# Keep-Passion/ImageStitch

Measured on AMD Instinct MI355X. Metric: image-pairs/sec (2048x2048 grayscale, SURF+BF), higher is better.
Workload: dtype f32

## Files before the change

### imagestitch_amd/csrc/surf_kernels.hip

```cpp
#include "common.h"
#include "detmath.h"
#include <math.h>
#include <float.h>
#include <string.h>
#include <stdlib.h>
#include <algorithm>
#include <vector>

#define GAS __attribute__((address_space(1)))
typedef GAS const uint8_t *g_cu8;
typedef GAS const int32_t *g_ci32;
typedef GAS float *g_f32;
typedef GAS const float *g_cf32;
typedef GAS int32_t *g_i32;
__device__ __forceinline__ int cv_round_f(float v) { return (int)rintf(v); }
__device__ __forceinline__ uint8_t round_u8_pos(float v) { return (uint8_t)__float_as_uint(v + 12582912.f); }
__device__ __forceinline__ int cv_round_d(double v) { return (int)rint(v); }
__device__ __forceinline__ int cv_floor_d(double v) { return (int)floor(v); }
__device__ __forceinline__ int cv_ceil_d(double v) { return (int)ceil(v); }

__device__ __forceinline__ int wave_incl_scan(int v)
{
    const int lane = threadIdx.x & 63;
#pragma unroll
// ... 730 lines not shown
        if (a1 > me.k1) rank++;
        else if (a1 == me.k1) {
            const unsigned long long a2 = S[q].k2, a3 = S[q].k3;
            rank += (a2 < me.k2 || (a2 == me.k2 && a3 < me.k3)) ? 1 : 0;
        }
    }
    const Cand c = R.cand[me.idx];
    vfsms_keypoint kp;
    kp.x = c.x; kp.y = c.y; kp.size = c.size; kp.angle = -1.f; kp.response = c.response;
    kp.octave = c.octave; kp.class_id = cand_class_id(R, pats, c);
    R.kps[rank] = kp;
}

__device__ __forceinline__ float fast_atan2_deg(float y, float x)
{
    const float s = (float)(180 / 3.1415926535897932384626433832795);
    const float p1 = 0.9997878412794807f * s, p3 = -0.3258083974640975f * s;
    const float p5 = 0.1555786518463281f * s, p7 = -0.04432655554792128f * s;
    float ax = fabsf(x), ay = fabsf(y);
    float a, c, c2;
    if (ax >= ay) {
        c = ay / (ax + (float)DBL_EPSILON);
        c2 = c * c;
        a = (((p7 * c2 + p5) * c2 + p3) * c2 + p1) * c;
    } else {
        c = ax / (ay + (float)DBL_EPSILON);
        c2 = c * c;
        a = 90.f - (((p7 * c2 + p5) * c2 + p3) * c2 + p1) * c;
    }
    if (x < 0) a = 180.f - a;
    if (y < 0) a = 360.f - a;
    return a;
}

#ifndef ORI_KP
#define ORI_KP 2
#endif
typedef float ori_f2 __attribute__((ext_vector_type(2)));
__device__ __forceinline__ void orientation_block(const RoiDev &R, const SurfTables *T, const int k0, const int n, int upright)
{
    __shared__ __attribute__((aligned(16))) float2 XY[ORI_KP][128];
    __shared__ __attribute__((aligned(16))) uint8_t Zb[ORI_KP][9][128];
    __shared__ float mod_s[ORI_KP][72], sx_s[ORI_KP][72], sy_s[ORI_KP][72];
    __shared__ int nvalid[ORI_KP], state[ORI_KP];
    const int tid = threadIdx.x;
    const int kq = __builtin_amdgcn_readfirstlane(tid >> 7), t = tid & 127;
    if (tid < ORI_KP) { nvalid[tid] = 0; state[tid] = 0; }
    __syncthreads();
    {
        const int k = k0 + kq;
        int valid = 0;
        uint32_t m0 = 0, m1 = 0, m2 = 0;
        float2 xy = make_float2(0.f, 0.f);
        if (k < n) {
            const vfsms_keypoint kp = R.kps[k];
            const float s = kp.size * 1.2f / 9.0f;
            const int gws = 2 * cv_round_f(2 * s);
            const int srows = R.h + 1, scols = R.w + 1, sw = R.w + 1;
            if (srows < gws || scols < gws) {
                if (t == 0) { R.kps[k].size = -1.f; state[kq] = 1; }
            } else if (upright) {
                if (t == 0) { R.kps[k].angle = 270.f; state[kq] = 1; }
            } else if (t < T->nOriSamples) {
                int x = cv_round_f(kp.x + T->aptx[t] * s - (float)(gws - 1) / 2);
                int y = cv_round_f(kp.y + T->apty[t] * s - (float)(gws - 1) / 2);
                if (!(y < 0 || y >= srows - gws || x < 0 || x >= scols - gws)) {
                    const float ratio = (float)gws / 4;
                    const int r2 = cv_round_f(ratio * 2), r4 = cv_round_f(ratio * 4);
                    g_ci32 p0 = (g_ci32)R.sum + (size_t)y * sw + x;
                    g_ci32 p2 = p0 + (size_t)r2 * sw, p4 = p0 + (size_t)r4 * sw;
                    const int a00 = p0[0], a02 = p0[r2], a04 = p0[r4];
                    const int a20 = p2[0], a24 = p2[r4];
                    const int a40 = p4[0], a42 = p4[r2], a44 = p4[r4];
                    const float wA = 1.f / ((float)r2 * (float)r4);
                    float wB = wA;
                    if (r4 - r2 != r2) wB = 1.f / ((float)(r4 - r2) * (float)r4);
                    const int vx0 = a00 + a42 - a40 - a02, vx1 = a02 + a44 - a42 - a04;
                    const int vy0 = a00 + a24 - a20 - a04, vy1 = a20 + a44 - a40 - a24;
                    double dxd = 0; dxd += (double)(-((float)vx0 * wA)); dxd += (double)((float)vx1 * wB);
                    double dyd = 0; dyd += (double)((float)vy0 * wA); dyd += (double)(-((float)vy1 * wB));
                    const float vx = (float)dxd, vy = (float)dyd;
                    const float aw = T->aptw[t];
                    const float xx = vx * aw, yy = vy * aw;
                    xy = make_float2(xx, yy);
                    const int ang = cv_round_f(fast_atan2_deg(yy, xx));
                    const uint32_t *mrow = T->oriMask[min(max(ang, 0), 360)];
                    m0 = mrow[0]; m1 = mrow[1]; m2 = mrow[2];
                    valid = 1;
                }
            }
        } else if (t == 0) state[kq] = 1;
        XY[kq][t] = xy;
        Zb[kq][0][t] = (uint8_t)m0; Zb[kq][1][t] = (uint8_t)(m0 >> 8); Zb[kq][2][t] = (uint8_t)(m0 >> 16); Zb[kq][3][t] = (uint8_t)(m0 >> 24);
        Zb[kq][4][t] = (uint8_t)m1; Zb[kq][5][t] = (uint8_t)(m1 >> 8); Zb[kq][6][t] = (uint8_t)(m1 >> 16); Zb[kq][7][t] = (uint8_t)(m1 >> 24);
        Zb[kq][8][t] = (uint8_t)m2;
        const unsigned long long m = __ballot(valid);
        if ((tid & 63) == 0 && m) atomicAdd(&nvalid[kq], __popcll(m));
    }
    __syncthreads();
    if (tid < ORI_KP * 72) {
        const int q = tid / 72, w = tid - q * 72;
        if (state[q] == 0 && nvalid[q] > 0) {
            const int nori = T->nOriSamples;
            const uint8_t *zrow = Zb[q][w >> 3];
            const int bit = w & 7;
            ori_f2 acc = {0.f, 0.f};
            for (int j = 0; j < nori; j += 8) {
                const uint2 z8 = *reinterpret_cast<const uint2 *>(&zrow[j]);
                const uint32_t za = (z8.x >> bit) & 0x01010101u, zb = (z8.y >> bit) & 0x01010101u;
                const float4 p01 = *reinterpret_cast<const float4 *>(&XY[q][j]), p23 = *reinterpret_cast<const float4 *>(&XY[q][j + 2]);
                const float4 p45 = *reinterpret_cast<const float4 *>(&XY[q][j + 4]), p67 = *reinterpret_cast<const float4 *>(&XY[q][j + 6]);
#define ORI_ACC(Z, N, P, XC, YC) do { float mf; asm("v_cvt_f32_ubyte" #N " %0, %1" : "=v"(mf) : "v"(Z)); \
                                           acc = __builtin_elementwise_fma((ori_f2){P.XC, P.YC}, (ori_f2){mf, mf}, acc); } while (0)
                ORI_ACC(za, 0, p01, x, y); ORI_ACC(za, 1, p01, z, w); ORI_ACC(za, 2, p23, x, y); ORI_ACC(za, 3, p23, z, w);
                ORI_ACC(zb, 0, p45, x, y); ORI_ACC(zb, 1, p45, z, w); ORI_ACC(zb, 2, p67, x, y); ORI_ACC(zb, 3, p67, z, w);
#undef ORI_ACC
            }
            const float sumx = acc.x, sumy = acc.y;
            mod_s[q][w] = sumx * sumx + sumy * sumy;
            sx_s[q][w] = sumx; sy_s[q][w] = sumy;
        }
    }
    __syncthreads();
    {
        const int q = __builtin_amdgcn_readfirstlane(tid >> 6), lane = tid & 63;
        if (q < ORI_KP && state[q] == 0) {
            const int k = k0 + q;
            if (nvalid[q] == 0) {
                if (lane == 0) R.kps[k].size = -1.f;
            } else {
                float bm = mod_s[q][lane]; int bi = lane;
                if (!(bm > 0.f)) bm = 0.f;
                if (lane < 8) { float m2 = mod_s[q][64 + lane]; if (m2 > bm) { bm = m2; bi = 64 + lane; } }
#pragma unroll
                for (int off = 32; off >= 1; off >>= 1) {
                    const float om = __shfl_xor(bm, off, 64); const int oi = __shfl_xor(bi, off, 64);
                    if (om > bm || (om == bm && oi < bi)) { bm = om; bi = oi; }
                }
                if (lane == 0) {
                    float bestx = 0, besty = 0;
                    if (bm > 0.f) { bestx = sx_s[q][bi]; besty = sy_s[q][bi]; }
                    R.kps[k].angle = fast_atan2_deg(-besty, bestx);
                }
            }
        }
    }
}

#ifdef VFSMS_DESC_TIMING
__device__ unsigned long long g_desc_cycles[8];
#define DT_MARK(ph) do { if (threadIdx.x == 0) { unsigned long long _n = clock64(); atomicAdd(&g_desc_cycles[ph], _n - _t0); _t0 = _n; } } while (0)
#define DT_START unsigned long long _t0 = clock64()
extern "C" int vfsms_debug_desc_cycles(unsigned long long *out) { return hipMemcpyFromSymbol(out, HIP_SYMBOL(g_desc_cycles), sizeof(unsigned long long) * 8) == hipSuccess ? 0 : -3; }
__device__ unsigned long long g_desc_trips[4];
#define DT_TRIP(n) do {} while (0)
__device__ unsigned long long g_desc_unit_cycles[4];
#define DT_UNIT_BEGIN unsigned long long _u0 = clock64()
#define DT_UNIT_END(n) do { _uacc[n] += clock64() - _u0; _ucnt[n]++; } while (0)
extern "C" int vfsms_debug_desc_unit_cycles(unsigned long long *out) { return hipMemcpyFromSymbol(out, HIP_SYMBOL(g_desc_unit_cycles), sizeof(unsigned long long) * 4) == hipSuccess ? 0 : -3; }
extern "C" int vfsms_debug_desc_trips(unsigned long long *out) { return hipMemcpyFromSymbol(out, HIP_SYMBOL(g_desc_trips), sizeof(unsigned long long) * 4) == hipSuccess ? 0 : -3; }
#else
#define DT_MARK(ph) do {} while (0)
#define DT_START do {} while (0)
#define DT_TRIP(n) do {} while (0)
#define DT_UNIT_BEGIN do {} while (0)
#define DT_UNIT_END(n) do {} while (0)
#endif
#ifndef VFSMS_EXP
#define VFSMS_EXP 0
#endif
#ifndef DESC_WBUF
#define DESC_WBUF 15360
#endif
__device__ __forceinline__ void origin_chain(float *row, float s, const float d, const int n)
{
    int i = 0;
    for (; i + 4 <= n; i += 4) {
        const float a = s, b = a + d, c = b + d, e = c + d;
        s = e + d;
        row[i] = a; row[i + 1] = b; row[i + 2] = c; row[i + 3] = e;
    }
    for (; i < n; i++, s += d) row[i] = s;
}

struct WinGeom {
    int win; float sin_dir, cos_dir;
    int h, w, stride; g_cu8 img;
    g_cu8 pair;
    int upright, usx, usy;
};

__device__ __forceinline__ int win_sample_xy(const WinGeom &G, double px, double py)
{
    const int ncols1 = G.w - 1, nrows1 = G.h - 1;
    const int ix = (int)px, iy = (int)py;
    if (px >= 0.0 && py >= 0.0 && ix < ncols1 && iy < nrows1) {
        const float a = (float)__builtin_amdgcn_fract(px), b = (float)__builtin_amdgcn_fract(py);
        g_cu8 p = G.img + (size_t)iy * G.stride + ix;
        const float v = p[0] * (1.f - a) * (1.f - b) + p[1] * a * (1.f - b) + p[G.stride] * (1.f - a) * b + p[G.stride + 1] * a * b;
        return (int)(uint8_t)cv_round_f(v);
    }
    const int x = min(max(cv_round_d(px), 0), ncols1);
    const int y = min(max(cv_round_d(py), 0), nrows1);
    return (int)G.img[(size_t)y * G.stride + x];
}
__device__ __forceinline__ int win_sample_upright(const WinGeom &G, int i, int j)
{
    const int x = min(max(G.usx + i, 0), G.w - 1);
    const int y = min(max(G.usy - j, 0), G.h - 1);
    return (int)G.img[(size_t)y * G.stride + x];
}

typedef float float2v __attribute__((ext_vector_type(2)));
__device__ __forceinline__ float bilinear_pk(uint32_t top, float a, float b)
{
    const float na = 1.f - a, nb = 1.f - b;
    const float2v w = {na, a};
    const float2v r0 = {(float)(top & 0xff), (float)((top >> 16) & 0xff)};
    const float2v r1 = {(float)((top >> 8) & 0xff), (float)(top >> 24)};
    float2v p = r0 * w, q = r1 * w;
    const float2v nb2 = {nb, nb}, b2 = {b, b};
    p = p * nb2; q = q * b2;
    return ((p.x + p.y) + q.x) + q.y;
}
#ifndef STAGE_ILP
#define STAGE_ILP 4
#endif
#define UNIT_W (8 * STAGE_ILP)
#ifndef BORDER_ILP
#define BORDER_ILP 2
#endif
#ifndef STAGE_FRAC_FIRST
#define STAGE_FRAC_FIRST 1
#endif
template <int N>
__device__ __forceinline__ void stage_round(g_cu8 ubase, const uint32_t pw, const double c, const double sn, const double sxc, const double syc,
                                            const int jlane, uint8_t *wrow)
{
    uint32_t top[N];
    const double jd = (double)jlane;
    const double px0 = __builtin_fma(jd, c, sxc), py0 = __builtin_fma(jd, -sn, syc);
#if STAGE_FRAC_FIRST
    float fa[N], fb[N];
#pragma unroll
    for (int u = 0; u < N; u++) {
        const double px = u ? px0 + (double)(8 * u) * c : px0, py = u ? py0 - (double)(8 * u) * sn : py0;
        const uint32_t off = ((uint32_t)__umul24((uint32_t)(int)py, pw) + (uint32_t)(int)px) << 1;
        fa[u] = (float)__builtin_amdgcn_fract(px); fb[u] = (float)__builtin_amdgcn_fract(py);
        top[u] = *(GAS const uint32_t *)(ubase + off);
    }
#pragma unroll
    for (int u = 0; u < N; u++) wrow[8 * u] = round_u8_pos(bilinear_pk(top[u], fa[u], fb[u]));
#else
    double px[N], py[N];
    px[0] = px0; py[0] = py0;
#pragma unroll
    for (int u = 1; u < N; u++) { px[u] = px[0] + (double)(8 * u) * c; py[u] = py[0] - (double)(8 * u) * sn; }
#pragma unroll
    for (int u = 0; u < N; u++) {
        const uint32_t off = ((uint32_t)__umul24((uint32_t)(int)py[u], pw) + (uint32_t)(int)px[u]) << 1;
        top[u] = *(GAS const uint32_t *)(ubase + off);
    }
#pragma unroll
    for (int u = 0; u < N; u++) {
        const float a = (float)__builtin_amdgcn_fract(px[u]), b = (float)__builtin_amdgcn_fract(py[u]);
        wrow[8 * u] = round_u8_pos(bilinear_pk(top[u], a, b));
    }
#endif
}

template <int NW>
__device__ __forceinline__ void stage_rows(const WinGeom &G, const float *sx_row, const float *sy_row,
                                           int r0, int nrows, uint8_t *dst, uint8_t *strip_in)
{
    const int win = __builtin_amdgcn_readfirstlane(G.win);
    r0 = __builtin_amdgcn_readfirstlane(r0); nrows = __builtin_amdgcn_readfirstlane(nrows);
    const int lane = threadIdx.x & 63, wv = NW == 1 ? 0 : __builtin_amdgcn_readfirstlane((int)(threadIdx.x >> 6));
    const int li = lane >> 3, lj = lane & 7;
    const int strips = (nrows + 7) >> 3;
    const double c = (double)G.cos_dir, sn = (double)G.sin_dir;
    const int ncols1 = __builtin_amdgcn_readfirstlane(G.w) - 1, nrows1 = __builtin_amdgcn_readfirstlane(G.h) - 1;
    const uint64_t bp = (uint64_t)G.pair;
    g_cu8 ubase = (g_cu8)(((uint64_t)(uint32_t)__builtin_amdgcn_readfirstlane((uint32_t)(bp >> 32)) << 32) |
                          (uint64_t)(uint32_t)__builtin_amdgcn_readfirstlane((uint32_t)bp));
    const uint32_t pw = (uint32_t)(ncols1 + 1);
    const int gfull = win >> 3, tailc = win & 7;
    int nb = NW == 1 ? 1 : (gfull + 7) >> 3;
#if VFSMS_EXP & 16
    nb = (gfull + 3) >> 2;
#endif
    const int gbase = gfull / nb, grem = gfull - gbase * nb;
    const int total = strips * nb;
    if (!G.upright) {
        const int tid = NW == 1 ? lane : (int)threadIdx.x;
        if (tid < strips) {
            const int ia = min(r0 + tid * 8, VFSMS_MAX_WIN - 1), ib = min(min(r0 + tid * 8 + 7, r0 + nrows - 1), VFSMS_MAX_WIN - 1);
            const double xa = (double)sx_row[ia], xb = (double)sx_row[ib], ya = (double)sy_row[ia], yb = (double)sy_row[ib];
            const double jb = (double)(win - 1);
            const double jxb = jb * c, jyb = -(jb * sn);
            const double xmin = fmin(xa, xb) + fmin(0.0, jxb), xmax = fmax(xa, xb) + fmax(0.0, jxb);
            const double ymin = fmin(ya, yb) + fmin(0.0, jyb), ymax = fmax(ya, yb) + fmax(0.0, jyb);
            strip_in[tid] = xmin >= 0.0 && ymin >= 0.0 && xmax < (double)(ncols1 - 2) && ymax < (double)nrows1;
        }
        if (NW == 1) { __builtin_amdgcn_fence(__ATOMIC_ACQ_REL, "wavefront"); __builtin_amdgcn_wave_barrier(); }
        else __syncthreads();
    }
    int ty = 0, cbi = wv;
    while (cbi >= nb) { cbi -= nb; ty++; }
#ifdef VFSMS_DESC_TIMING
    unsigned long long _s0 = clock64(), _uacc[2] = {0, 0}, _ucnt[2] = {0, 0};
#endif
    const int last_row = r0 + nrows - 1;
    const int liw = li * win;
    const int last_off = (nrows - 1) * win;
    float nsx = 0.f, nsy = 0.f; int nflag = 0;
    if (wv < total) {
        const int ic0 = min(r0 + ty * 8 + li, last_row);
        nsx = sx_row[ic0]; nsy = sy_row[ic0]; nflag = strip_in[ty];
    }
    for (int unit = wv; unit < total; unit += NW) {
        DT_UNIT_BEGIN;
        const int g0 = cbi * gbase + min(cbi, grem), gn = gbase + (cbi < grem ? 1 : 0);
        const bool last_run = cbi == nb - 1;
        const int cb0 = g0 * 8;
        const int cb1 = last_run ? win : cb0 + gn * 8;
        const double sxc = (double)nsx, syc = (double)nsy;
        const int flag_cur = nflag;
        const int ty_cur = ty;
        uint8_t *drc = dst + min(ty * 8 * win + liw, last_off);
        cbi += NW;
        while (cbi >= nb) { cbi -= nb; ty++; }
        if (unit + NW < total) {
            const int icn = min(r0 + ty * 8 + li, last_row);
            nsx = sx_row[icn]; nsy = sy_row[icn]; nflag = strip_in[ty];
        }
        if (G.upright) {
            for (int j = cb0 + lj; j < cb1; j += 8) drc[j] = (uint8_t)win_sample_upright(G, min(r0 + ty_cur * 8 + li, last_row), j);
            continue;
        }
        bool unit_in = __builtin_amdgcn_readfirstlane(flag_cur) != 0;
        if (!unit_in) {
            const int ia = min(r0 + ty_cur * 8, VFSMS_MAX_WIN - 1), ib = min(min(r0 + ty_cur * 8 + 7, last_row), VFSMS_MAX_WIN - 1);
            const double xa = (double)sx_row[ia], xb = (double)sx_row[ib], ya = (double)sy_row[ia], yb = (double)sy_row[ib];
            const double ja = (double)cb0, jb = (double)(cb1 - 1);
            const double jxa = ja * c, jxb = jb * c, jya = -(ja * sn), jyb = -(jb * sn);
            const double xmin = fmin(xa, xb) + fmin(jxa, jxb), xmax = fmax(xa, xb) + fmax(jxa, jxb);
            const double ymin = fmin(ya, yb) + fmin(jya, jyb), ymax = fmax(ya, yb) + fmax(jya, jyb);
            unit_in = xmin >= 0.0 && ymin >= 0.0 && xmax < (double)(ncols1 - 2) && ymax < (double)nrows1;
        }
        if (unit_in) {
            DT_TRIP(0);
            uint8_t *wrow = drc + cb0 + lj;
            int jl = cb0 + lj, left = gn;
            while (left >= 4) { stage_round<4>(ubase, pw, c, sn, sxc, syc, jl, wrow); jl += 32; wrow += 32; left -= 4; }
            if (left == 3) stage_round<3>(ubase, pw, c, sn, sxc, syc, jl, wrow);
            else if (left == 2) stage_round<2>(ubase, pw, c, sn, sxc, syc, jl, wrow);
            else if (left == 1) stage_round<1>(ubase, pw, c, sn, sxc, syc, jl, wrow);
            if (last_run && tailc) {
                const int jc = min(gfull * 8 + lj, win - 1);
                stage_round<1>(ubase, pw, c, sn, sxc, syc, jc, drc + jc);
            }
            DT_UNIT_END(0);
            continue;
        }
        DT_TRIP(2);
        for (int jb = cb0; jb < cb1; jb += 8 * BORDER_ILP) {
            double px[BORDER_ILP], py[BORDER_ILP];
            int jc[BORDER_ILP];
            uint32_t top[BORDER_ILP];
            bool inside[BORDER_ILP];
#pragma unroll
            for (int u = 0; u < BORDER_ILP; u++) {
                jc[u] = min(jb + u * 8 + lj, cb1 - 1);
                px[u] = sxc + (double)jc[u] * c;
                py[u] = syc - (double)jc[u] * sn;
                const int ix = (int)px[u], iy = (int)py[u];
                inside[u] = px[u] >= 0.0 && py[u] >= 0.0 && ix < ncols1 && iy < nrows1;
                const int rx = min(max(cv_round_d(px[u]), 0), ncols1), ry = min(max(cv_round_d(py[u]), 0), nrows1);
                const int cx = inside[u] ? ix : rx, cy = inside[u] ? iy : ry;
                top[u] = *(GAS const uint32_t *)(ubase + (((uint32_t)__umul24((uint32_t)cy, pw) + (uint32_t)cx) << 1));
            }
#pragma unroll
            for (int u = 0; u < BORDER_ILP; u++) {
                const float a = (float)__builtin_amdgcn_fract(px[u]), b = (float)__builtin_amdgcn_fract(py[u]);
                const float v = (float)(top[u] & 0xff) * (1.f - a) * (1.f - b) + (float)((top[u] >> 16) & 0xff) * a * (1.f - b) +
                                (float)((top[u] >> 8) & 0xff) * (1.f - a) * b + (float)(top[u] >> 24) * a * b;
                drc[jc[u]] = inside[u] ? (uint8_t)cv_round_f(v) : (uint8_t)(top[u] & 0xff);
            }
        }
        DT_UNIT_END(1);
    }
#ifdef VFSMS_DESC_TIMING
    if ((threadIdx.x & 63) == 0) {
        atomicAdd(&g_desc_unit_cycles[2], clock64() - _s0);
        atomicAdd(&g_desc_unit_cycles[0], _uacc[0]); atomicAdd(&g_desc_unit_cycles[1], _uacc[1]);
        atomicAdd(&g_desc_trips[0], _ucnt[0]); atomicAdd(&g_desc_trips[2], _ucnt[1]);
    }
#endif
}

__device__ __forceinline__ uint8_t sat_u8(float v)
{
    int iv = cv_round_f(v);
    return (uint8_t)(iv < 0 ? 0 : iv > 255 ? 255 : iv);
}

struct AreaRec { int j0, n; float a0, af, al; int mode, r1, r2; };
#define AREA_RECS 22

__device__ __forceinline__ float area_row_tab(const uint8_t *S, const AreaRec &c, const int nmin, const int nmax)
{
    const uint8_t *p = S + c.j0;
    float buf = (float)p[0] * c.a0;
    int t = 1;
    for (; t < nmin - 1; t++) buf += (float)p[t] * c.af;
    for (; t < nmax; t++) buf += (float)p[t] * (t < c.n - 1 ? c.af : (t == c.n - 1 ? c.al : 0.f));
    return buf;
}
#define AREA_TAIL 4
__device__ __forceinline__ void area_tail_weights(const AreaRec &c, const int nmin, float (&w)[AREA_TAIL])
{
    const int t0 = max(nmin - 1, 1);
#pragma unroll
    for (int i = 0; i < AREA_TAIL; i++) w[i] = t0 + i < c.n - 1 ? c.af : (t0 + i == c.n - 1 ? c.al : 0.f);
}
__device__ __forceinline__ float area_row_tab_w(const uint8_t *S, const AreaRec &c, const int nmin, const int nmax, const float (&w)[AREA_TAIL])
{
    const uint8_t *p = S + c.j0;
    float buf = (float)p[0] * c.a0;
    int t = 1;
    for (; t < nmin - 1; t++) buf += (float)p[t] * c.af;
#pragma unroll
    for (int i = 0; i < AREA_TAIL; i++)
        if (t + i < nmax) buf += (float)p[t + i] * w[i];
    return buf;
}
__device__ __forceinline__ uint8_t area_out(const float sum, const int mode, const float inv_area)
{
    if (mode == 2) return (uint8_t)(((int)sum + 2) >> 2);
    if (mode == 1) return sat_u8(sum * inv_area);
    return sat_u8(sum);
}
__device__ __forceinline__ uint8_t area_col_tab(const float *rb, const AreaRec &c, const int mode, const float inv_area)
{
    float sum = c.a0 * rb[0];
    for (int t = 1; t < c.n; t++) sum += (t < c.n - 1 ? c.af : c.al) * rb[t * 21];
    return area_out(sum, mode, inv_area);
}
#define DESC_ACC_OFF (DESC_WBUF - 441 * 4)
#define DESC_PASS 36

__device__ void describe_one(const RoiDev &R, const SurfTables *T, const AreaRec *area_tab, const DescRec &rec, int extended, int upright, const int band)
{
    DT_START;
    const int k = rec.k;
    __shared__ float sx_row[VFSMS_MAX_WIN], sy_row[VFSMS_MAX_WIN];
    __shared__ uint8_t PATCH[21][21 + 3];
    __shared__ AreaRec REC[AREA_RECS];
    __shared__ uint8_t WINBUF[DESC_WBUF];
    __shared__ float rowsum[40 * 21];
    __shared__ uint8_t STRIP_IN[VFSMS_MAX_WIN / 8 + 8];
    WinGeom G;
    G.win = max(21, min(rec.win, VFSMS_MAX_WIN));
    G.h = R.h; G.w = R.w; G.stride = R.stride; G.img = (g_cu8)R.img; G.pair = (g_cu8)R.pair;
    G.upright = upright; G.usx = 0; G.usy = 0; G.sin_dir = rec.sin_dir; G.cos_dir = rec.cos_dir;
    const int win = G.win;
    const int dsz = 21;
    if (threadIdx.x < AREA_RECS * 8) ((int *)REC)[threadIdx.x] = ((const int *)(area_tab + (size_t)win * AREA_RECS))[threadIdx.x];
    __syncthreads();
    const int nmin = __builtin_amdgcn_readfirstlane(REC[21].j0), nmax = __builtin_amdgcn_readfirstlane(REC[21].n);
    const int mode = __builtin_amdgcn_readfirstlane(REC[21].mode);
    const float inv_area = REC[21].a0;
    if (!upright) {
        if (threadIdx.x == 0 || threadIdx.x == 64) {
            const float sin_dir = rec.sin_dir, cos_dir = rec.cos_dir;
            const float win_offset = -(float)(win - 1) / 2;
            const int need = band >= 0 ? min(win, REC[band].j0 + REC[band].n) : win;
            if (threadIdx.x == 0) origin_chain(sx_row, rec.x + win_offset * cos_dir + win_offset * sin_dir, sin_dir, need);
            else origin_chain(sy_row, rec.y - win_offset * sin_dir + win_offset * cos_dir, cos_dir, need);
        }
    } else {
        const float win_offset = -(float)(win - 1) / 2;
        G.usx = cv_round_f(rec.x + win_offset);
        G.usy = cv_round_f(rec.y - win_offset);
    }
    __syncthreads();
    DT_MARK(0);

    const bool tail_ok = nmax - max(nmin - 1, 1) <= AREA_TAIL;
    auto reduce_rows = [&](const int st_lo, int dyA, const int dy_stop) {
        while (dyA < dy_stop) {
            const int lo = REC[dyA].j0;
            int dyB = dyA + 1;
            while (dyB < dy_stop && REC[dyB].j0 + REC[dyB].n - lo <= 40) dyB++;
            const int nr = REC[dyB - 1].j0 + REC[dyB - 1].n - lo;
            for (int e = threadIdx.x; e < nr * 21; e += 256) {
                const int r = (int)(((uint32_t)e * 3121u) >> 16), dx = e - 21 * r;
                if (tail_ok) {
                    const AreaRec cx = REC[dx];
                    float w[AREA_TAIL];
                    area_tail_weights(cx, nmin, w);
                    rowsum[e] = area_row_tab_w(WINBUF + (lo - st_lo + r) * win, cx, nmin, nmax, w);
                } else
                    rowsum[e] = area_row_tab(WINBUF + (lo - st_lo + r) * win, REC[dx], nmin, nmax);
            }
            __syncthreads();
            for (int o = threadIdx.x; o < (dyB - dyA) * 21; o += 256) {
                const int dyl = (int)(((uint32_t)o * 3121u) >> 16), dx = o - 21 * dyl;
                const AreaRec ry = REC[dyA + dyl];
                PATCH[dyA + dyl][dx] = area_col_tab(rowsum + (ry.j0 - lo) * 21 + dx, ry, mode, inv_area);
            }
            __syncthreads();
            dyA = dyB;
        }
    };
    if (win * win <= DESC_WBUF) {
        stage_rows<4>(G, sx_row, sy_row, 0, win, WINBUF, STRIP_IN);
        __syncthreads();
        DT_MARK(1);
        reduce_rows(0, 0, dsz);
        DT_MARK(2);
    } else {
        float *acc = (float *)(WINBUF + DESC_ACC_OFF);
        const int dyA = band >= 0 ? band : 0, dyB = band >= 0 ? band + 1 : dsz;
        const int rlo = REC[dyA].j0, rhi = REC[dyB - 1].j0 + REC[dyB - 1].n;
        const int crows = (DESC_ACC_OFF / win) & ~7;
        for (int c0 = rlo; c0 < rhi; c0 += crows) {
            const int cn = min(crows, rhi - c0);
            stage_rows<4>(G, sx_row, sy_row, c0, cn, WINBUF, STRIP_IN);
            __syncthreads();
            DT_MARK(3);
            for (int p0 = 0; p0 < cn; p0 += DESC_PASS) {
                const int pn = min(DESC_PASS, cn - p0);
                for (int e = threadIdx.x; e < pn * 21; e += 256) {
                    const int r = (int)(((uint32_t)e * 3121u) >> 16), dx = e - 21 * r;
                    if (tail_ok) {
                        const AreaRec cx = REC[dx];
                        float w[AREA_TAIL];
                        area_tail_weights(cx, nmin, w);
                        rowsum[e] = area_row_tab_w(WINBUF + (p0 + r) * win, cx, nmin, nmax, w);
                    } else
                        rowsum[e] = area_row_tab(WINBUF + (p0 + r) * win, REC[dx], nmin, nmax);
                }
                __syncthreads();
                const int s0 = c0 + p0, s1 = s0 + pn;
                for (int o = threadIdx.x; o < 441; o += 256) {
                    const int dy = (int)(((uint32_t)o * 3121u) >> 16), dx = o - 21 * dy;
                    const AreaRec ry = REC[dy];
                    const int a = max(ry.j0, s0), b = min(ry.j0 + ry.n, s1);
                    if (dy < dyA || dy >= dyB || a >= b) continue;
                    float sum = a == ry.j0 ? 0.f : acc[o];
                    for (int s = a; s < b; s++) {
                        const int t = s - ry.j0;
                        const float rb = rowsum[(s - s0) * 21 + dx];
                        if (t == 0) sum = ry.a0 * rb;
                        else sum += (t < ry.n - 1 ? ry.af : ry.al) * rb;
                    }
                    if (b == ry.j0 + ry.n) PATCH[dy][dx] = area_out(sum, mode, inv_area);
                    else acc[o] = sum;
                }
                if (p0 + DESC_PASS < cn) __syncthreads();
            }
            DT_MARK(4);
        }
    }
    __syncthreads();
    if (band >= 0) {
        if (threadIdx.x < 21) R.patch[(size_t)k * VFSMS_PATCH_ROW + band * 21 + threadIdx.x] = PATCH[band][threadIdx.x];
    } else {
        for (int o = threadIdx.x; o < 441; o += 256) R.patch[(size_t)k * VFSMS_PATCH_ROW + o] = PATCH[o / 21][o % 21];
    }
    DT_MARK(5);
}

#define DESC_NCLS 4

__device__ __forceinline__ int desc_class(float size)
{
    const float s = size * 1.2f / 9.0f;
    const int win = min((int)((20 + 1) * s), VFSMS_MAX_WIN);
    return win > 256 ? 0 : win > 128 ? 1 : win > 64 ? 2 : 3;
}

__global__ __launch_bounds__(1024) void k_desc_order(const RoiDev *rois)
{
    const RoiDev &R = rois[blockIdx.x];
    const int n = min(R.counters[0], R.cap);
    __shared__ int cnt[DESC_NCLS], base[DESC_NCLS], cur[DESC_NCLS];
    if (threadIdx.x < DESC_NCLS) { cnt[threadIdx.x] = 0; cur[threadIdx.x] = 0; }
    __syncthreads();
    const int lane = threadIdx.x & 63;
    for (int k0 = 0; k0 < n; k0 += 1024) {
        const int k = k0 + threadIdx.x;
        const float size = k < n ? R.kps[k].size : -1.f;
        const int cls = size > 0 ? desc_class(size) : -1;
#pragma unroll
        for (int c = 0; c < DESC_NCLS; c++) {
            const unsigned long long m = __ballot(cls == c);
            if (m && lane == __ffsll((long long)m) - 1) atomicAdd(&cnt[c], __popcll(m));
        }
    }
    __syncthreads();
    if (threadIdx.x == 0) {
        int acc = 0;
        for (int c = 0; c < DESC_NCLS; c++) { base[c] = acc; acc += cnt[c]; R.counters[12 + c] = cnt[c]; }
    }
    __syncthreads();
    for (int k0 = 0; k0 < n; k0 += 1024) {
        const int k = k0 + threadIdx.x;
        const float size = k < n ? R.kps[k].size : -1.f;
        const int cls = size > 0 ? desc_class(size) : -1;
#pragma unroll
        for (int c = 0; c < DESC_NCLS; c++) {
            const unsigned long long m = __ballot(cls == c);
            if (!m) continue;
            const int leader = __ffsll((long long)m) - 1;
            int start = 0;
            if (lane == leader) start = atomicAdd(&cur[c], __popcll(m));
            start = __shfl(start, leader, 64);
            if (cls == c) R.order[base[c] + start + __popcll(m & ((1ull << lane) - 1))] = k;
        }
    }
}

#define DESC_HEADS DESC_PLAN_HEADS
#define DESC_HEAD_STRIDE 64

__global__ __launch_bounds__(256) void k_desc_plan(const RoiDev *rois, int nrois, DescPlan *plan, int big_grid)
{
    __shared__ int c[VFSMS_MAX_ROIS][4];
    for (int e = threadIdx.x; e < nrois * 4; e += 256) c[e >> 2][e & 3] = rois[e >> 2].counters[12 + (e & 3)];
    __syncthreads();
    if (threadIdx.x == 0) {
        int acc = 0, total = 0;
        for (int q = 0; q < DESC_HEADS; q++) {
            plan->big_start[q] = acc;
            for (int r = q; r < nrois; r += DESC_HEADS) { plan->seg_base[r][0] = acc; acc += c[r][0]; }
            plan->big_n0[q] = acc - plan->big_start[q];
            for (int r = q; r < nrois; r += DESC_HEADS) {
                plan->seg_base[r][1] = acc; acc += c[r][1];
                plan->seg_base[r][2] = acc; acc += c[r][2];
            }
            plan->big_tickets[q] = acc - plan->big_start[q];
        }
        total = acc;
        const int split = total < big_grid * 48 ? 21 : 1;
        plan->split = split;
        for (int q = 0; q < DESC_HEADS; q++) plan->big_tickets[q] += (split - 1) * plan->big_n0[q];
        acc = 0;
        for (int q = 0; q < DESC_HEADS; q++) {
            plan->small_start[q] = acc;
            for (int r = q; r < nrois; r += DESC_HEADS) { plan->seg_base[r][3] = acc; acc += c[r][3]; }
            plan->small_tickets[q] = acc - plan->small_start[q];
        }
    }
}

__global__ __launch_bounds__(256) void k_desc_recs(const RoiDev *rois, const DescPlan *plan, DescRec *big, DescRec *small, int upright)
{
    const int roi = blockIdx.y;
    const RoiDev &R = rois[roi];
    const int p = blockIdx.x * 256 + threadIdx.x;
    const int c0 = R.counters[12], c1 = R.counters[13], c2 = R.counters[14], c3 = R.counters[15];
    if (p >= c0 + c1 + c2 + c3) return;
    const int cls = p < c0 ? 0 : p < c0 + c1 ? 1 : p < c0 + c1 + c2 ? 2 : 3;
    const int idx = p - (cls > 0 ? c0 : 0) - (cls > 1 ? c1 : 0) - (cls > 2 ? c2 : 0);
    const int k = R.order[p];
    const vfsms_keypoint kp = R.kps[k];
    DescRec rec;
    rec.roi = roi; rec.k = k; rec.pad = 0; rec.x = kp.x; rec.y = kp.y;
    rec.win = (int)((20 + 1) * (kp.size * 1.2f / 9.0f));
    rec.sin_dir = 0.f; rec.cos_dir = 0.f;
    if (!upright) {
        const float dir = kp.angle * (float)(3.1415926535897932384626433832795 / 180);
        double sd, cd;
        det_sincos((double)dir, &sd, &cd);
        rec.sin_dir = -(float)sd;
        rec.cos_dir = (float)cd;
    }
    (cls < 3 ? big : small)[plan->seg_base[roi][cls] + idx] = rec;
}

__global__ __launch_bounds__(ORI_KP * 128, 8) void k_orientation(const RoiDev *rois, const SurfTables *T, int upright)
{
    const RoiDev &R = rois[blockIdx.y];
    const int n = min(R.counters[0], R.cap);
    const int k0 = blockIdx.x * ORI_KP;
    if (k0 >= n) return;
    orientation_block(R, T, k0, n, upright);
}

#define DESC_SMALL_WIN 64
struct SmallLds { uint8_t win[DESC_SMALL_WIN * DESC_SMALL_WIN + 64]; float sx[DESC_SMALL_WIN + 8], sy[DESC_SMALL_WIN + 8]; AreaRec rec[AREA_RECS]; int rec_win; uint8_t strip_in[DESC_SMALL_WIN / 8 + 8]; };

__device__ __forceinline__ void wave_sync_lds()
{
    __builtin_amdgcn_fence(__ATOMIC_ACQ_REL, "wavefront");
    __builtin_amdgcn_wave_barrier();
}

__device__ void describe_small(const RoiDev &R, const AreaRec *area_tab, const DescRec &rec, int upright, SmallLds &L)
{
    const int lane = threadIdx.x & 63;
    const int k = rec.k;
    WinGeom G;
    G.win = min(rec.win, DESC_SMALL_WIN);
    G.h = R.h; G.w = R.w; G.stride = R.stride; G.img = (g_cu8)R.img; G.pair = (g_cu8)R.pair;
    G.upright = upright; G.usx = 0; G.usy = 0; G.sin_dir = rec.sin_dir; G.cos_dir = rec.cos_dir;
    const int win = G.win;
    const int dsz = 21;
    if (L.rec_win != win) {
        wave_sync_lds();
        const int *src = (const int *)(area_tab + (size_t)max(win, dsz) * AREA_RECS);
        for (int e = lane; e < AREA_RECS * 8; e += 64) ((int *)L.rec)[e] = src[e];
        if (lane == 0) L.rec_win = win;
    }
    if (!upright) {
        const float sin_dir = rec.sin_dir, cos_dir = rec.cos_dir;
        if (lane < 2) {
            const float win_offset = -(float)(win - 1) / 2;
            const float sx0 = rec.x + win_offset * cos_dir + win_offset * sin_dir, sy0 = rec.y - win_offset * sin_dir + win_offset * cos_dir;
            origin_chain(lane == 0 ? L.sx : L.sy, lane == 0 ? sx0 : sy0, lane == 0 ? sin_dir : cos_dir, win);
        }
    } else {
        const float win_offset = -(float)(win - 1) / 2;
        G.usx = cv_round_f(rec.x + win_offset);
        G.usy = cv_round_f(rec.y - win_offset);
    }
    wave_sync_lds();
    stage_rows<1>(G, L.sx, L.sy, 0, win, L.win, L.strip_in);
    wave_sync_lds();
    const int nmin = __builtin_amdgcn_readfirstlane(L.rec[21].j0), nmax = __builtin_amdgcn_readfirstlane(L.rec[21].n);
    const int mode = __builtin_amdgcn_readfirstlane(L.rec[21].mode);
    const float inv_area = L.rec[21].a0;
    const bool tail_ok = nmax - max(nmin - 1, 1) <= AREA_TAIL;
    uint8_t *prow = R.patch + (size_t)k * VFSMS_PATCH_ROW;
    for (int o = lane; o < dsz * dsz; o += 64) {
        const int dy = (int)(((uint32_t)o * 3121u) >> 16), dx = o - dsz * dy;
        const AreaRec ry = L.rec[dy], rx = L.rec[dx];
        const uint8_t *S = L.win + ry.j0 * win;
        float sum;
        if (tail_ok) {
            float w[AREA_TAIL];
            area_tail_weights(rx, nmin, w);
            sum = ry.a0 * area_row_tab_w(S, rx, nmin, nmax, w);
            for (int ty = 1; ty < nmax; ty++) {
                const float beta = ty < ry.n - 1 ? ry.af : (ty == ry.n - 1 ? ry.al : 0.f);
                sum += beta * area_row_tab_w(S + ty * win, rx, nmin, nmax, w);
            }
        } else {
            sum = ry.a0 * area_row_tab(S, rx, nmin, nmax);
            for (int ty = 1; ty < nmax; ty++) {
                const float beta = ty < ry.n - 1 ? ry.af : (ty == ry.n - 1 ? ry.al : 0.f);
                sum += beta * area_row_tab(S + ty * win, rx, nmin, nmax);
            }
        }
        uint8_t outv;
        if (mode == 2) outv = (uint8_t)(((int)sum + 2) >> 2);
        else if (mode == 1) outv = sat_u8(sum * inv_area);
        else outv = sat_u8(sum);
        prow[o] = outv;
    }
    wave_sync_lds();
}

#ifndef DESC_SMALL_WGS
#define DESC_SMALL_WGS 7
#endif
__device__ __forceinline__ DescRec load_rec_uniform(const DescRec *p)
{
    const int *q = (const int *)p;
    DescRec r;
    r.roi = __builtin_amdgcn_readfirstlane(q[0]); r.k = __builtin_amdgcn_readfirstlane(q[1]);
    r.win = __builtin_amdgcn_readfirstlane(q[2]); r.pad = 0;
    r.sin_dir = __int_as_float(__builtin_amdgcn_readfirstlane(q[4])); r.cos_dir = __int_as_float(__builtin_amdgcn_readfirstlane(q[5]));
    r.x = __int_as_float(__builtin_amdgcn_readfirstlane(q[6])); r.y = __int_as_float(__builtin_amdgcn_readfirstlane(q[7]));
    return r;
}
__global__ __launch_bounds__(256, DESC_SMALL_WGS) void k_describe_small(const RoiDev *rois, const DescPlan *plan, const DescRec *recs, int *counter,
                                                                 const AreaRec *area_tab, int upright)
{
    __shared__ SmallLds L[4];
    if (threadIdx.x < 4) L[threadIdx.x].rec_win = -1;
    __syncthreads();
    const int lane = threadIdx.x & 63, wave = __builtin_amdgcn_readfirstlane((int)(threadIdx.x >> 6));
    int head = 0;
    for (;;) {
        int slot = -1;
        if (lane == 0)
            while (head < DESC_HEADS) {
                const int q = (blockIdx.x + head) & (DESC_HEADS - 1);
                const int n = plan->small_tickets[q];
                const int t = n > 0 ? atomicAdd(counter + q * DESC_HEAD_STRIDE, 1) : 0;
                if (t < n) { slot = plan->small_start[q] + t; break; }
                head++;
            }
        slot = __builtin_amdgcn_readfirstlane(slot);
        head = __builtin_amdgcn_readfirstlane(head);
        if (slot < 0) break;
        const DescRec rec = load_rec_uniform(recs + slot);
        describe_small(rois[rec.roi], area_tab, rec, upright, L[wave]);
    }
}

__global__ __launch_bounds__(256) void k_pair_rows(const RoiDev *rois)
{
    const RoiDev &R = rois[blockIdx.z];
    const int y = blockIdx.y, x = (blockIdx.x * 256 + threadIdx.x) * 4;
    if (y >= R.h || x >= R.w) return;
    g_cu8 r0 = (g_cu8)R.img + (size_t)y * R.stride + x, r1 = (g_cu8)R.img + (size_t)min(y + 1, R.h - 1) * R.stride + x;
    GAS uint16_t *dst = (GAS uint16_t *)R.pair + (size_t)y * R.w + x;
    if (x + 4 <= R.w) {
        const uint32_t a = *(GAS const u32u *)r0, b = *(GAS const u32u *)r1;
#pragma unroll
        for (int k = 0; k < 4; k++) dst[k] = (uint16_t)(((a >> (8 * k)) & 0xff) | (((b >> (8 * k)) & 0xff) << 8));
    } else {
        for (int k = 0; x + k < R.w; k++) dst[k] = (uint16_t)(r0[k] | (r1[k] << 8));
    }
}

#ifndef DESC_WGS
#define DESC_WGS 6
#endif
__global__ __launch_bounds__(256, DESC_WGS) void k_describe(const RoiDev *rois, const DescPlan *plan, const DescRec *recs, int *counter, const SurfTables *T,
                                                  const AreaRec *area_tab, int extended, int upright)
{
    __shared__ int s_slot, s_band;
    int head = 0;
#ifdef VFSMS_DESC_TIMING
    unsigned long long tq = clock64();
#endif
    for (;;) {
        __syncthreads();
        if (threadIdx.x == 0) {
            int slot = -1, band = -1;
            const int split = plan->split;
            while (head < DESC_HEADS) {
                const int q = (blockIdx.x + head) & (DESC_HEADS - 1);
                const int n = plan->big_tickets[q];
                const int t = n > 0 ? atomicAdd(counter + q * DESC_HEAD_STRIDE, 1) : 0;
                if (t < n) {
                    const int n0 = plan->big_n0[q];
                    if (t < n0 * split) { slot = plan->big_start[q] + t / split; band = split > 1 ? t % split : -1; }
                    else slot = plan->big_start[q] + n0 + (t - n0 * split);
                    break;
                }
                head++;
            }
            s_slot = slot; s_band = band;
        }
        __syncthreads();
        const int slot = __builtin_amdgcn_readfirstlane(s_slot), band = __builtin_amdgcn_readfirstlane(s_band);
        if (slot < 0) break;
#ifdef VFSMS_DESC_TIMING
        if (threadIdx.x == 0) atomicAdd(&g_desc_cycles[6], clock64() - tq);
#endif
        const DescRec rec = load_rec_uniform(recs + slot);
        describe_one(rois[rec.roi], T, area_tab, rec, extended, upright, band);
#ifdef VFSMS_DESC_TIMING
        tq = clock64();
#endif
    }
}

__global__ __launch_bounds__(1024) void k_keep_scan(const RoiDev *rois)
{
    const RoiDev &R = rois[blockIdx.x];
    const int n = min(R.counters[0], R.cap);
    __shared__ int wsum[16];
    __shared__ int carry;
    if (threadIdx.x == 0) carry = 0;
    __syncthreads();
    const int lane = threadIdx.x & 63, wid = threadIdx.x >> 6;
    for (int base = 0; base < n; base += 1024) {
        int idx = base + threadIdx.x;
        int keep = (idx < n) ? (R.kps[idx].size > 0 ? 1 : 0) : 0;
        int incl = wave_incl_scan(keep);
        if (lane == 63) wsum[wid] = incl;
        __syncthreads();
        int off = carry;
        for (int k = 0; k < wid; k++) off += wsum[k];
        if (idx < n) R.keep_pos[idx] = keep ? (off + incl - 1) : -1;
        __syncthreads();
// ... 301 lines not shown
```

Baseline: 2337.

## Classify each 8x8 staging group as inside, outside or border for rotated windows

Replaces the per-strip inside flag with a per-(strip, column-group) classification computed up front. Within each unit, a ballot over the group classes dispatches runs of groups to the fast bilinear path, to a cheap nearest-clamped path for fully outside groups, or to the per-pixel border path. The aim is to keep the fast vectorised path for interior parts of strips that touch the image border, and to skip bilinear work on out-of-image pixels. In exchange it adds LDS for the class table, more prologue work and a more divergent per-unit loop. The table size is capped at STAGE_CLS_MAX entries, which may be too small for large windows.

```diff
diff --git a/imagestitch_amd/csrc/surf_kernels.hip b/imagestitch_amd/csrc/surf_kernels.hip
--- a/imagestitch_amd/csrc/surf_kernels.hip
+++ b/imagestitch_amd/csrc/surf_kernels.hip
@@ -906,19 +906,21 @@
 #define DT_MARK(ph) do { if (threadIdx.x == 0) { unsigned long long _n = clock64(); atomicAdd(&g_desc_cycles[ph], _n - _t0); _t0 = _n; } } while (0)
 #define DT_START unsigned long long _t0 = clock64()
 extern "C" int vfsms_debug_desc_cycles(unsigned long long *out) { return hipMemcpyFromSymbol(out, HIP_SYMBOL(g_desc_cycles), sizeof(unsigned long long) * 8) == hipSuccess ? 0 : -3; }
-__device__ unsigned long long g_desc_trips[4];
-#define DT_TRIP(n) do {} while (0)
-__device__ unsigned long long g_desc_unit_cycles[4];
+__device__ unsigned long long g_desc_trips[2][4];
+__device__ unsigned long long g_desc_unit_cycles[2][4];
+__device__ unsigned long long g_desc_groups[2][4];
 #define DT_UNIT_BEGIN unsigned long long _u0 = clock64()
 #define DT_UNIT_END(n) do { _uacc[n] += clock64() - _u0; _ucnt[n]++; } while (0)
-extern "C" int vfsms_debug_desc_unit_cycles(unsigned long long *out) { return hipMemcpyFromSymbol(out, HIP_SYMBOL(g_desc_unit_cycles), sizeof(unsigned long long) * 4) == hipSuccess ? 0 : -3; }
-extern "C" int vfsms_debug_desc_trips(unsigned long long *out) { return hipMemcpyFromSymbol(out, HIP_SYMBOL(g_desc_trips), sizeof(unsigned long long) * 4) == hipSuccess ? 0 : -3; }
+#define DT_GROUPS(kind, n) do { _gcnt[kind] += (n); } while (0)
+extern "C" int vfsms_debug_desc_unit_cycles(unsigned long long *out) { return hipMemcpyFromSymbol(out, HIP_SYMBOL(g_desc_unit_cycles), sizeof(unsigned long long) * 8) == hipSuccess ? 0 : -3; }
+extern "C" int vfsms_debug_desc_trips(unsigned long long *out) { return hipMemcpyFromSymbol(out, HIP_SYMBOL(g_desc_trips), sizeof(unsigned long long) * 8) == hipSuccess ? 0 : -3; }
+extern "C" int vfsms_debug_desc_groups(unsigned long long *out) { return hipMemcpyFromSymbol(out, HIP_SYMBOL(g_desc_groups), sizeof(unsigned long long) * 8) == hipSuccess ? 0 : -3; }
 #else
 #define DT_MARK(ph) do {} while (0)
 #define DT_START do {} while (0)
-#define DT_TRIP(n) do {} while (0)
 #define DT_UNIT_BEGIN do {} while (0)
 #define DT_UNIT_END(n) do {} while (0)
+#define DT_GROUPS(kind, n) do {} while (0)
 #endif
 #ifndef VFSMS_EXP
 #define VFSMS_EXP 0
@@ -980,10 +982,8 @@
 #ifndef STAGE_ILP
 #define STAGE_ILP 4
 #endif
+#define STAGE_CLS_MAX 256
 #define UNIT_W (8 * STAGE_ILP)
-#ifndef BORDER_ILP
-#define BORDER_ILP 2
-#endif
 #ifndef STAGE_FRAC_FIRST
 #define STAGE_FRAC_FIRST 1
 #endif
@@ -1023,9 +1023,51 @@
 #endif
 }
 
+template <int N>
+__device__ __forceinline__ void stage_nearest(g_cu8 ubase, const uint32_t pw, const double c, const double sn, const double sxc, const double syc,
+                                              const int jlane, uint8_t *wrow, const int ncols1, const int nrows1)
+{
+    uint8_t v[N];
+#pragma unroll
+    for (int u = 0; u < N; u++) {
+        const double jd = (double)(jlane + 8 * u);
+        const double px = sxc + jd * c, py = syc - jd * sn;
+        const int rx = min(max(cv_round_d(px), 0), ncols1), ry = min(max(cv_round_d(py), 0), nrows1);
+        v[u] = *(ubase + (((uint32_t)__umul24((uint32_t)ry, pw) + (uint32_t)rx) << 1));
+    }
+#pragma unroll
+    for (int u = 0; u < N; u++) wrow[8 * u] = v[u];
+}
+template <int N>
+__device__ __forceinline__ void stage_border(g_cu8 ubase, const uint32_t pw, const double c, const double sn, const double sxc, const double syc,
+                                             const int jlane, uint8_t *wrow, const int ncols1, const int nrows1)
+{
+    double px[N], py[N];
+    uint32_t top[N];
+    bool inside[N];
+#pragma unroll
+    for (int u = 0; u < N; u++) {
+        const double jd = (double)(jlane + 8 * u);
+        px[u] = sxc + jd * c;
+        py[u] = syc - jd * sn;
+        const int ix = (int)px[u], iy = (int)py[u];
+        inside[u] = px[u] >= 0.0 && py[u] >= 0.0 && ix < ncols1 && iy < nrows1;
+        const int rx = min(max(cv_round_d(px[u]), 0), ncols1), ry = min(max(cv_round_d(py[u]), 0), nrows1);
+        const int cx = inside[u] ? ix : rx, cy = inside[u] ? iy : ry;
+        top[u] = *(GAS const uint32_t *)(ubase + (((uint32_t)__umul24((uint32_t)cy, pw) + (uint32_t)cx) << 1));
+    }
+#pragma unroll
+    for (int u = 0; u < N; u++) {
+        const float a = (float)__builtin_amdgcn_fract(px[u]), b = (float)__builtin_amdgcn_fract(py[u]);
+        const float v = (float)(top[u] & 0xff) * (1.f - a) * (1.f - b) + (float)((top[u] >> 16) & 0xff) * a * (1.f - b) +
+                        (float)((top[u] >> 8) & 0xff) * (1.f - a) * b + (float)(top[u] >> 24) * a * b;
+        wrow[8 * u] = inside[u] ? (uint8_t)cv_round_f(v) : (uint8_t)(top[u] & 0xff);
+    }
+}
+
 template <int NW>
 __device__ __forceinline__ void stage_rows(const WinGeom &G, const float *sx_row, const float *sy_row,
-                                           int r0, int nrows, uint8_t *dst, uint8_t *strip_in)
+                                           int r0, int nrows, uint8_t *dst, uint8_t *group_cls)
 {
     const int win = __builtin_amdgcn_readfirstlane(G.win);
     r0 = __builtin_amdgcn_readfirstlane(r0); nrows = __builtin_amdgcn_readfirstlane(nrows);
@@ -1045,16 +1087,21 @@
 #endif
     const int gbase = gfull / nb, grem = gfull - gbase * nb;
     const int total = strips * nb;
+    const int ngr = gfull + (tailc ? 1 : 0);
     if (!G.upright) {
         const int tid = NW == 1 ? lane : (int)threadIdx.x;
-        if (tid < strips) {
-            const int ia = min(r0 + tid * 8, VFSMS_MAX_WIN - 1), ib = min(min(r0 + tid * 8 + 7, r0 + nrows - 1), VFSMS_MAX_WIN - 1);
+        const float rngr = __builtin_amdgcn_rcpf((float)ngr);
+        for (int e = tid; e < strips * ngr; e += NW * 64) {
+            const int s = (int)(((float)e + 0.5f) * rngr), g = e - s * ngr;
+            const int ia = min(r0 + s * 8, VFSMS_MAX_WIN - 1), ib = min(min(r0 + s * 8 + 7, r0 + nrows - 1), VFSMS_MAX_WIN - 1);
             const double xa = (double)sx_row[ia], xb = (double)sx_row[ib], ya = (double)sy_row[ia], yb = (double)sy_row[ib];
-            const double jb = (double)(win - 1);
-            const double jxb = jb * c, jyb = -(jb * sn);
-            const double xmin = fmin(xa, xb) + fmin(0.0, jxb), xmax = fmax(xa, xb) + fmax(0.0, jxb);
-            const double ymin = fmin(ya, yb) + fmin(0.0, jyb), ymax = fmax(ya, yb) + fmax(0.0, jyb);
-            strip_in[tid] = xmin >= 0.0 && ymin >= 0.0 && xmax < (double)(ncols1 - 2) && ymax < (double)nrows1;
+            const double ja = (double)(g * 8), jb = (double)min(g * 8 + 7, win - 1);
+            const double jxa = ja * c, jxb = jb * c, jya = -(ja * sn), jyb = -(jb * sn);
+            const double xmin = fmin(xa, xb) + fmin(jxa, jxb), xmax = fmax(xa, xb) + fmax(jxa, jxb);
+            const double ymin = fmin(ya, yb) + fmin(jya, jyb), ymax = fmax(ya, yb) + fmax(jya, jyb);
+            const bool in = xmin >= 0.0 && ymin >= 0.0 && xmax < (double)(ncols1 - 2) && ymax < (double)nrows1;
+            const bool out = xmax < 0.0 || ymax < 0.0 || xmin >= (double)ncols1 || ymin >= (double)nrows1;
+            group_cls[e] = in ? 1 : out ? 2 : 0;
         }
         if (NW == 1) { __builtin_amdgcn_fence(__ATOMIC_ACQ_REL, "wavefront"); __builtin_amdgcn_wave_barrier(); }
         else __syncthreads();
@@ -1062,93 +1109,85 @@
     int ty = 0, cbi = wv;
     while (cbi >= nb) { cbi -= nb; ty++; }
 #ifdef VFSMS_DESC_TIMING
-    unsigned long long _s0 = clock64(), _uacc[2] = {0, 0}, _ucnt[2] = {0, 0};
+    unsigned long long _s0 = clock64(), _uacc[2] = {0, 0}, _ucnt[2] = {0, 0}, _gcnt[3] = {0, 0, 0};
 #endif
     const int last_row = r0 + nrows - 1;
     const int liw = li * win;
     const int last_off = (nrows - 1) * win;
-    float nsx = 0.f, nsy = 0.f; int nflag = 0;
+    float nsx = 0.f, nsy = 0.f; int ncl = 0;
     if (wv < total) {
         const int ic0 = min(r0 + ty * 8 + li, last_row);
-        nsx = sx_row[ic0]; nsy = sy_row[ic0]; nflag = strip_in[ty];
+        nsx = sx_row[ic0]; nsy = sy_row[ic0];
+        ncl = group_cls[ty * ngr + min(cbi * gbase + min(cbi, grem) + (lane & 15), ngr - 1)];
     }
     for (int unit = wv; unit < total; unit += NW) {
         DT_UNIT_BEGIN;
         const int g0 = cbi * gbase + min(cbi, grem), gn = gbase + (cbi < grem ? 1 : 0);
         const bool last_run = cbi == nb - 1;
         const int cb0 = g0 * 8;
-        const int cb1 = last_run ? win : cb0 + gn * 8;
         const double sxc = (double)nsx, syc = (double)nsy;
-        const int flag_cur = nflag;
+        const int cl_cur = ncl;
         const int ty_cur = ty;
         uint8_t *drc = dst + min(ty * 8 * win + liw, last_off);
         cbi += NW;
         while (cbi >= nb) { cbi -= nb; ty++; }
         if (unit + NW < total) {
             const int icn = min(r0 + ty * 8 + li, last_row);
-            nsx = sx_row[icn]; nsy = sy_row[icn]; nflag = strip_in[ty];
+            nsx = sx_row[icn]; nsy = sy_row[icn];
+            ncl = group_cls[ty * ngr + min(cbi * gbase + min(cbi, grem) + (lane & 15), ngr - 1)];
         }
         if (G.upright) {
+            const int cb1 = last_run ? win : cb0 + gn * 8;
             for (int j = cb0 + lj; j < cb1; j += 8) drc[j] = (uint8_t)win_sample_upright(G, min(r0 + ty_cur * 8 + li, last_row), j);
             continue;
         }
-        bool unit_in = __builtin_amdgcn_readfirstlane(flag_cur) != 0;
-        if (!unit_in) {
-            const int ia = min(r0 + ty_cur * 8, VFSMS_MAX_WIN - 1), ib = min(min(r0 + ty_cur * 8 + 7, last_row), VFSMS_MAX_WIN - 1);
-            const double xa = (double)sx_row[ia], xb = (double)sx_row[ib], ya = (double)sy_row[ia], yb = (double)sy_row[ib];
-            const double ja = (double)cb0, jb = (double)(cb1 - 1);
-            const double jxa = ja * c, jxb = jb * c, jya = -(ja * sn), jyb = -(jb * sn);
-            const double xmin = fmin(xa, xb) + fmin(jxa, jxb), xmax = fmax(xa, xb) + fmax(jxa, jxb);
-            const double ymin = fmin(ya, yb) + fmin(jya, jyb), ymax = fmax(ya, yb) + fmax(jya, jyb);
-            unit_in = xmin >= 0.0 && ymin >= 0.0 && xmax < (double)(ncols1 - 2) && ymax < (double)nrows1;
-        }
-        if (unit_in) {
-            DT_TRIP(0);
-            uint8_t *wrow = drc + cb0 + lj;
-            int jl = cb0 + lj, left = gn;
-            while (left >= 4) { stage_round<4>(ubase, pw, c, sn, sxc, syc, jl, wrow); jl += 32; wrow += 32; left -= 4; }
-            if (left == 3) stage_round<3>(ubase, pw, c, sn, sxc, syc, jl, wrow);
-            else if (left == 2) stage_round<2>(ubase, pw, c, sn, sxc, syc, jl, wrow);
-            else if (left == 1) stage_round<1>(ubase, pw, c, sn, sxc, syc, jl, wrow);
-            if (last_run && tailc) {
-                const int jc = min(gfull * 8 + lj, win - 1);
-                stage_round<1>(ubase, pw, c, sn, sxc, syc, jc, drc + jc);
-            }
-            DT_UNIT_END(0);
-            continue;
-        }
-        DT_TRIP(2);
-        for (int jb = cb0; jb < cb1; jb += 8 * BORDER_ILP) {
-            double px[BORDER_ILP], py[BORDER_ILP];
-            int jc[BORDER_ILP];
-            uint32_t top[BORDER_ILP];
-            bool inside[BORDER_ILP];
-#pragma unroll
-            for (int u = 0; u < BORDER_ILP; u++) {
-                jc[u] = min(jb + u * 8 + lj, cb1 - 1);
-                px[u] = sxc + (double)jc[u] * c;
-                py[u] = syc - (double)jc[u] * sn;
-                const int ix = (int)px[u], iy = (int)py[u];
-                inside[u] = px[u] >= 0.0 && py[u] >= 0.0 && ix < ncols1 && iy < nrows1;
-                const int rx = min(max(cv_round_d(px[u]), 0), ncols1), ry = min(max(cv_round_d(py[u]), 0), nrows1);
-                const int cx = inside[u] ? ix : rx, cy = inside[u] ? iy : ry;
-                top[u] = *(GAS const uint32_t *)(ubase + (((uint32_t)__umul24((uint32_t)cy, pw) + (uint32_t)cx) << 1));
-            }
-#pragma unroll
-            for (int u = 0; u < BORDER_ILP; u++) {
-                const float a = (float)__builtin_amdgcn_fract(px[u]), b = (float)__builtin_amdgcn_fract(py[u]);
-                const float v = (float)(top[u] & 0xff) * (1.f - a) * (1.f - b) + (float)((top[u] >> 16) & 0xff) * a * (1.f - b) +
-                                (float)((top[u] >> 8) & 0xff) * (1.f - a) * b + (float)(top[u] >> 24) * a * b;
-                drc[jc[u]] = inside[u] ? (uint8_t)cv_round_f(v) : (uint8_t)(top[u] & 0xff);
-            }
-        }
-        DT_UNIT_END(1);
+        const bool tail = last_run && tailc;
+        const uint32_t inm = (uint32_t)__ballot(cl_cur == 1) & 0xffffu, outm = (uint32_t)__ballot(cl_cur == 2) & 0xffffu;
+        const int jl = cb0 + lj;
+        uint8_t *wrow = drc + jl;
+        int g = 0;
+        while (g < gn) {
+            int n = min(__builtin_ctz(~(inm >> g)), gn - g);
+            if (n > 0) {
+                DT_GROUPS(0, min(n, 4));
+                if (n >= 4) { stage_round<4>(ubase, pw, c, sn, sxc, syc, jl + 8 * g, wrow + 8 * g); g += 4; }
+                else if (n == 3) { stage_round<3>(ubase, pw, c, sn, sxc, syc, jl + 8 * g, wrow + 8 * g); g += 3; }
+                else if (n == 2) { stage_round<2>(ubase, pw, c, sn, sxc, syc, jl + 8 * g, wrow + 8 * g); g += 2; }
+                else { stage_round<1>(ubase, pw, c, sn, sxc, syc, jl + 8 * g, wrow + 8 * g); g += 1; }
+                continue;
+            }
+            n = min(__builtin_ctz(~(outm >> g)), gn - g);
+            if (n > 0) {
+                if (n >= 4) { stage_nearest<4>(ubase, pw, c, sn, sxc, syc, jl + 8 * g, wrow + 8 * g, ncols1, nrows1); n = 4; }
+                else if (n >= 2) { stage_nearest<2>(ubase, pw, c, sn, sxc, syc, jl + 8 * g, wrow + 8 * g, ncols1, nrows1); n = 2; }
+                else stage_nearest<1>(ubase, pw, c, sn, sxc, syc, jl + 8 * g, wrow + 8 * g, ncols1, nrows1);
+                DT_GROUPS(2, n);
+                g += n;
+                continue;
+            }
+            if (g + 1 < gn && !(((inm | outm) >> (g + 1)) & 1)) { stage_border<2>(ubase, pw, c, sn, sxc, syc, jl + 8 * g, wrow + 8 * g, ncols1, nrows1); n = 2; }
+            else { stage_border<1>(ubase, pw, c, sn, sxc, syc, jl + 8 * g, wrow + 8 * g, ncols1, nrows1); n = 1; }
+            DT_GROUPS(1, n);
+            g += n;
+        }
+        if (tail) {
+            const int jc = min(gfull * 8 + lj, win - 1);
+            if ((inm >> gn) & 1) { DT_GROUPS(0, 1); stage_round<1>(ubase, pw, c, sn, sxc, syc, jc, drc + jc); }
+            else if ((outm >> gn) & 1) { DT_GROUPS(2, 1); stage_nearest<1>(ubase, pw, c, sn, sxc, syc, jc, drc + jc, ncols1, nrows1); }
+            else { DT_GROUPS(1, 1); stage_border<1>(ubase, pw, c, sn, sxc, syc, jc, drc + jc, ncols1, nrows1); }
+        }
+#ifdef VFSMS_DESC_TIMING
+        const uint32_t _all = (1u << (gn + (tail ? 1 : 0))) - 1u;
+        if ((inm & _all) == _all) DT_UNIT_END(0); else DT_UNIT_END(1);
+#endif
     }
 #ifdef VFSMS_DESC_TIMING
     if ((threadIdx.x & 63) == 0) {
-        atomicAdd(&g_desc_unit_cycles[2], clock64() - _s0);
-        atomicAdd(&g_desc_unit_cycles[0], _uacc[0]); atomicAdd(&g_desc_unit_cycles[1], _uacc[1]);
-        atomicAdd(&g_desc_trips[0], _ucnt[0]); atomicAdd(&g_desc_trips[2], _ucnt[1]);
+        const int cls = win > 123;
+        atomicAdd(&g_desc_unit_cycles[cls][2], clock64() - _s0);
+        atomicAdd(&g_desc_unit_cycles[cls][0], _uacc[0]); atomicAdd(&g_desc_unit_cycles[cls][1], _uacc[1]);
+        atomicAdd(&g_desc_trips[cls][0], _ucnt[0]); atomicAdd(&g_desc_trips[cls][2], _ucnt[1]);
+        for (int q = 0; q < 3; q++) atomicAdd(&g_desc_groups[cls][q], _gcnt[q]);
     }
 #endif
 }
@@ -1213,7 +1252,7 @@
     __shared__ AreaRec REC[AREA_RECS];
     __shared__ uint8_t WINBUF[DESC_WBUF];
     __shared__ float rowsum[40 * 21];
-    __shared__ uint8_t STRIP_IN[VFSMS_MAX_WIN / 8 + 8];
+    __shared__ uint8_t GROUP_CLS[STAGE_CLS_MAX];
     WinGeom G;
     G.win = max(21, min(rec.win, VFSMS_MAX_WIN));
     G.h = R.h; G.w = R.w; G.stride = R.stride; G.img = (g_cu8)R.img; G.pair = (g_cu8)R.pair;
@@ -1269,7 +1308,7 @@
         }
     };
     if (win * win <= DESC_WBUF) {
-        stage_rows<4>(G, sx_row, sy_row, 0, win, WINBUF, STRIP_IN);
+        stage_rows<4>(G, sx_row, sy_row, 0, win, WINBUF, GROUP_CLS);
         __syncthreads();
         DT_MARK(1);
         reduce_rows(0, 0, dsz);
@@ -1281,7 +1320,7 @@
         const int crows = (DESC_ACC_OFF / win) & ~7;
         for (int c0 = rlo; c0 < rhi; c0 += crows) {
             const int cn = min(crows, rhi - c0);
-            stage_rows<4>(G, sx_row, sy_row, c0, cn, WINBUF, STRIP_IN);
+            stage_rows<4>(G, sx_row, sy_row, c0, cn, WINBUF, GROUP_CLS);
             __syncthreads();
             DT_MARK(3);
             for (int p0 = 0; p0 < cn; p0 += DESC_PASS) {
@@ -1445,7 +1484,7 @@
 }
 
 #define DESC_SMALL_WIN 64
-struct SmallLds { uint8_t win[DESC_SMALL_WIN * DESC_SMALL_WIN + 64]; float sx[DESC_SMALL_WIN + 8], sy[DESC_SMALL_WIN + 8]; AreaRec rec[AREA_RECS]; int rec_win; uint8_t strip_in[DESC_SMALL_WIN / 8 + 8]; };
+struct SmallLds { uint8_t win[DESC_SMALL_WIN * DESC_SMALL_WIN + 64]; float sx[DESC_SMALL_WIN + 8], sy[DESC_SMALL_WIN + 8]; AreaRec rec[AREA_RECS]; int rec_win; uint8_t group_cls[(DESC_SMALL_WIN / 8) * (DESC_SMALL_WIN / 8)]; };
 
 __device__ __forceinline__ void wave_sync_lds()
 {
@@ -1482,7 +1521,7 @@
         G.usy = cv_round_f(rec.y - win_offset);
     }
     wave_sync_lds();
-    stage_rows<1>(G, L.sx, L.sy, 0, win, L.win, L.strip_in);
+    stage_rows<1>(G, L.sx, L.sy, 0, win, L.win, L.group_cls);
     wave_sync_lds();
     const int nmin = __builtin_amdgcn_readfirstlane(L.rec[21].j0), nmax = __builtin_amdgcn_readfirstlane(L.rec[21].n);
     const int mode = __builtin_amdgcn_readfirstlane(L.rec[21].mode);
```

Result: no change. 2338, median of 2 (+0.0%).
